# qucontrol/krotov

Hardware: AMD Instinct MI355X
Metric: state*timestep propagations/s (Krotov iterations/s in iterations_per_sec), 256-objective N=64 ensemble (higher is better)
Workload: dtype f64

## Files before the change

krotov_amd/csrc/kh_tile64q2.h:

```cpp
#pragma once

#include "kh_common.h"
#include "kh_generic.h"
#include "kh_tile64.h"

#define KH_Q2_THREADS 512
#ifdef KH_Q2_DPP_REDUCE
typedef KhLanes<false> KhQ2Lanes;
#else
typedef KhLanes<true> KhQ2Lanes;
#endif
#define KH_Q2_TILE_ELEMS (8 * KH_Q2_THREADS)

#ifdef KH_Q2_LDS_BROADCAST
constexpr bool KH_Q2_R16 = false;
#else
constexpr bool KH_Q2_R16 = true;
#endif

template <bool R16>
struct KhQ2Map;
template <>
struct KhQ2Map<false> {
    static __device__ __forceinline__ int half(int) { return 0; }
    static __device__ __forceinline__ int row_in(int wave, int lane) { return wave * 8 + KhQ2Lanes::row_in(lane); }
    static __device__ __forceinline__ int col(int, int lane, int j) { return KhQ2Lanes::cg(lane) + 8 * j; }
    static __device__ __forceinline__ int row_out(int wave, int lane) { return wave * 8 + KhQ2Lanes::row_out(lane); }
    static __device__ __forceinline__ bool writer(int lane) { return (lane & 7) == 0; }
    static __device__ __forceinline__ double rowsum(double v, double scale) { return KhQ2Lanes::rowsum(v, scale); }
};
template <>
struct KhQ2Map<true> {
    static __device__ __forceinline__ int half(int wave) { return KhLanesR16::half(wave); }
    static __device__ __forceinline__ int row_in(int wave, int lane) { return KhLanesR16::row_in(wave, lane); }
    static __device__ __forceinline__ int col(int wave, int lane, int j) { return KhLanesR16::col0(wave, lane) + j; }
    static __device__ __forceinline__ int row_out(int wave, int lane) { return KhLanesR16::row_out(wave, lane); }
    static __device__ __forceinline__ bool writer(int lane) { return KhLanesR16::writer(lane); }
    static __device__ __forceinline__ double rowsum(double v, double scale) { return KhLanesR16::rowsum(v, scale); }
};

struct KhQ2Lds {
    cplx *h0;
    cplx *p0;
    cplx (*buf)[2][KH_TILE_N];
    cplx *chib;
    cplx (*sbuf)[KH_TILE_N];
    double *red;
    double *D;
    double2 *inv2;
    double *deg;
};

__host__ __device__ inline size_t kh_q2_lds_bytes() {
    return (size_t)2 * KH_Q2_TILE_ELEMS * sizeof(cplx) + 7 * KH_TILE_N * sizeof(cplx) + (2 * 8 * 2 + 4) * sizeof(double) +
           (KH_MAX_DEGREE / 2 + 1) * sizeof(double2) + (KH_MAX_DEGREE + 2) * sizeof(double);
}

__device__ __forceinline__ KhQ2Lds kh_q2_carve(char *smem) {
    KhQ2Lds s;
    s.h0 = (cplx *)smem;
    s.p0 = s.h0 + KH_Q2_TILE_ELEMS;
    s.buf = (cplx(*)[2][KH_TILE_N])(s.p0 + KH_Q2_TILE_ELEMS);
    s.chib = (cplx *)(s.buf + 2);
    s.sbuf = (cplx(*)[KH_TILE_N])(s.chib + KH_TILE_N);
    s.red = (double *)(s.sbuf + 2);
    s.D = s.red + 2 * 8 * 2;
    s.inv2 = (double2 *)(s.D + 4);
    s.deg = (double *)(s.inv2 + KH_MAX_DEGREE / 2 + 1);
    return s;
}

template <bool R16>
__device__ __forceinline__ void kh_q2_load_tile(const cplx *op, int N, int wave, int lane, cplx (&t)[8]) {
    const int row = KhQ2Map<R16>::row_in(wave, lane);
#pragma unroll
    for (int j = 0; j < 8; ++j) {
        const int col = KhQ2Map<R16>::col(wave, lane, j);
        t[j] = (op != nullptr && row < N && col < N) ? op[(size_t)row * N + col] : c_make(0.0, 0.0);
    }
}

template <bool R16>
__device__ __forceinline__ void kh_q2_stage_tile(const cplx *op, int N, int wave, int lane, int tid, cplx *dst) {
    cplx t[8];
    kh_q2_load_tile<R16>(op, N, wave, lane, t);
#pragma unroll
    for (int j = 0; j < 8; ++j) dst[j * KH_Q2_THREADS + tid] = t[j];
}

__device__ __forceinline__ void kh_q2_load_rows(const KhSweepArgs &p, const KhQ2Lds &s, int m, int tid) {
    __syncthreads();
    if (tid < KH_Q2_ROWS) {
        const double *r = p.q2_rows + ((size_t)m * KH_Q2_ROWS + tid) * 2;
        s.inv2[tid] = make_double2(r[0], r[1]);
    }
    if (tid == KH_Q2_ROWS) s.inv2[KH_Q2_ROWS] = make_double2(p.q2_c0[m], 0.0);
    __syncthreads();
}

template <bool R16>
__device__ __forceinline__ cplx kh_q2_dot(const cplx (&t)[8], const cplx *x0, const cplx *x1, int wave, int lane) {
    cplx acc = c_make(0.0, 0.0);
    if constexpr (R16) {
        const int xi = KhLanesR16::x_index(wave, lane);
        const cplx xa = x0[xi], xb = x1[xi];
        KhLanesR16::dot8(acc, t, c_make(xa.x + xb.x, xa.y + xb.y));
    } else {
        const int cg = KhQ2Lanes::cg(lane);
        cplx xv[8];
#pragma unroll
        for (int j = 0; j < 8; ++j) xv[j] = x0[cg + 8 * j];
#pragma unroll
        for (int j = 0; j < 8; ++j) c_fma(acc, t[j], xv[j]);
    }
    return acc;
}
template <bool R16>
__device__ __forceinline__ cplx kh_q2_vec_at(const cplx (*v)[KH_TILE_N], int i) {
    cplx x = v[0][i];
    if constexpr (R16) {
        x.x += v[1][i].x;
        x.y += v[1][i].y;
    }
    return x;
}

__device__ __forceinline__ void kh_q2_build(const KhQ2Lds &s, int tid, double eps, const cplx (&h1)[8],
                                            const cplx (&p1)[8], const cplx (&p2)[8], cplx (&a)[8], cplx (&b)[8]) {
    const double eps2 = eps * eps;
#pragma unroll
    for (int j = 0; j < 8; ++j) {
        const cplx h0 = s.h0[j * KH_Q2_THREADS + tid];
        const cplx q0 = s.p0[j * KH_Q2_THREADS + tid];
        a[j].x = fma(eps, h1[j].x, h0.x);
        a[j].y = fma(eps, h1[j].y, h0.y);
        b[j].x = fma(eps2, p2[j].x, fma(eps, p1[j].x, q0.x));
        b[j].y = fma(eps2, p2[j].y, fma(eps, p1[j].y, q0.y));
    }
}

#define KH_Q2_REFRESH 64
__device__ __forceinline__ void kh_q2_restart_lds(const KhQ2Lds &s, int tid, cplx (&a)[8], cplx (&b)[8]) {
#pragma unroll
    for (int j = 0; j < 8; ++j) {
        a[j] = s.h0[j * KH_Q2_THREADS + tid];
        b[j] = s.p0[j * KH_Q2_THREADS + tid];
    }
}
__device__ __forceinline__ void kh_q2_advance_reg(double eps, double eps_prev, const cplx (&h1)[8], const cplx (&p1)[8],
                                                  const cplx (&p2)[8], cplx (&a)[8], cplx (&b)[8]) {
    const double e1 = eps - eps_prev, e2 = e1 * (eps + eps_prev);
#pragma unroll
    for (int j = 0; j < 8; ++j) {
        a[j].x = fma(e1, h1[j].x, a[j].x);
        a[j].y = fma(e1, h1[j].y, a[j].y);
        b[j].x = fma(e2, p2[j].x, fma(e1, p1[j].x, b[j].x));
        b[j].y = fma(e2, p2[j].y, fma(e1, p1[j].y, b[j].y));
    }
}

__device__ __forceinline__ void kh_q2_advance(const KhQ2Lds &s, int tid, double eps, double eps_prev, const cplx (&h1)[8],
                                              cplx (&a)[8], cplx (&b)[8]) {
    const double e1 = eps - eps_prev, e2 = e1 * (eps + eps_prev);
#pragma unroll
    for (int j = 0; j < 8; ++j) {
        const cplx q1 = s.h0[j * KH_Q2_THREADS + tid];
        const cplx q2 = s.p0[j * KH_Q2_THREADS + tid];
        a[j].x = fma(e1, h1[j].x, a[j].x);
        a[j].y = fma(e1, h1[j].y, a[j].y);
        b[j].x = fma(e2, q2.x, fma(e1, q1.x, b[j].x));
        b[j].y = fma(e2, q2.y, fma(e1, q1.y, b[j].y));
    }
}

template <bool R16, class Epilogue>
__device__ __forceinline__ int kh_q2_expm_action(const cplx (&a)[8], const cplx (&b)[8], cplx &state,
                                                 cplx (*buf)[2][KH_TILE_N], cplx (*sbuf)[KH_TILE_N], const double2 *inv2,
                                                 int &cur, cplx *store_in, int N, double fre, double fim,
                                                 double dt, int nsub, int m, bool odd, int wave, int lane,
                                                 Epilogue epilogue) {
    typedef KhQ2Map<R16> Map;
    const int row = Map::row_out(wave, lane), half = Map::half(wave);
    const bool writer = Map::writer(lane);
    const double h = nsub == 1 ? dt : dt / nsub;
    const double f2h2 = (fre * fre - fim * fim) * h * h;
    const int phases = (m + 1) >> 1;
    const bool no_last_b = odd && (m & 1);
    if (store_in != nullptr && wave == 0 && lane < N) {
        store_in[lane] = kh_q2_vec_at<R16>(buf[cur], lane);
    }
    for (int sub = 0; sub < nsub; ++sub) {
        const double hr = h * inv2[0].x, c0 = inv2[KH_Q2_ROWS].x;
        cplx sacc = c_make(hr * state.x, hr * state.y);
        state = c_make(c0 * state.x, c0 * state.y);
        if (phases == 1) {
            if (writer) sbuf[half][row] = sacc;
            __syncthreads();
        }
        for (int ph = 0; ph < phases; ++ph) {
            const bool last = (ph + 1 == phases);
            if (!(last && no_last_b)) {
                double c2, hn = 0.0;
                cplx yb;
                if constexpr (R16) {
                    const int xi = KhLanesR16::x_index(wave, lane);
                    const cplx x0 = buf[cur][0][xi], x1 = buf[cur][1][xi];
                    const double r2 = inv2[ph].y, r1n = inv2[ph + 1].x;
                    c2 = f2h2 * r2;
                    hn = h * r1n;
                    yb = c_make(0.0, 0.0);
                    KhLanesR16::dot8(yb, b, c_make(x0.x + x1.x, x0.y + x1.y));
                } else {
                    c2 = f2h2 * inv2[ph].y;
                    yb = kh_q2_dot<R16>(b, buf[cur][0], buf[cur][1], wave, lane);
                }
                const double t2x = Map::rowsum(yb.x, c2), t2y = Map::rowsum(yb.y, c2);
                state.x += t2x;
                state.y += t2y;
                if (!last) {
                    if constexpr (!R16) hn = h * inv2[ph + 1].x;
                    sacc.x = fma(hn, t2x, sacc.x);
                    sacc.y = fma(hn, t2y, sacc.y);
                    if (writer) {
                        buf[cur ^ 1][half][row] = c_make(t2x, t2y);
                        if (ph + 2 == phases) sbuf[half][row] = sacc;
                    }
                }
            }
            if (last) {
                __builtin_amdgcn_sched_barrier(0);
                const cplx ya = kh_q2_dot<R16>(a, sbuf[0], sbuf[1], wave, lane);
                const cplx odd_sum = c_mul(c_make(fre, fim), c_make(Map::rowsum(ya.x, 1.0), Map::rowsum(ya.y, 1.0)));
                state.x += odd_sum.x;
                state.y += odd_sum.y;
                if (writer) buf[cur ^ 1][half][row] = c_make(state.x, state.y);
                if (sub + 1 == nsub) epilogue();
            }
            __syncthreads();
            cur ^= 1;
        }
    }
    return nsub * (phases + (no_last_b ? 0 : 1));
}

template <bool R16>
__device__ __forceinline__ void kh_q2_sweep_store_body(const KhSweepArgs &p, const cplx *const *__restrict__ sq,
                                                       const double *__restrict__ pulses,
                                                       const cplx *__restrict__ state_in, cplx *__restrict__ store,
                                                       cplx *__restrict__ state_out, int direction, char *smem) {
    const KhQ2Lds s = kh_q2_carve(smem);
    const int tid = threadIdx.x, wave = tid >> 6, lane = tid & 63;
    if (tid <= KH_MAX_DEGREE) s.deg[tid] = p.q2_theta[tid];
    typedef KhQ2Map<R16> Map;
    const int row = Map::row_out(wave, lane);
    const int half = Map::half(wave);
    const bool writer = Map::writer(lane);
    const int N = p.N, nt = p.nt;
    double matvecs = 0.0;
    for (int k = blockIdx.x; k < p.K; k += gridDim.x) {
        const cplx *const *ops_k = p.ops + (size_t)k * 2;
        const cplx *const *sq_k = sq + (size_t)k * 3;
        __syncthreads();
        kh_q2_stage_tile<R16>(ops_k[0], N, wave, lane, tid, s.h0);
        kh_q2_stage_tile<R16>(sq_k[0], N, wave, lane, tid, s.p0);
        cplx h1[8], p1[8], p2[8];
        kh_q2_load_tile<R16>(ops_k[1], N, wave, lane, h1);
        kh_q2_load_tile<R16>(sq_k[1], N, wave, lane, p1);
        kh_q2_load_tile<R16>(sq_k[2], N, wave, lane, p2);
        const double nrm0 = p.op_norms[(size_t)k * 2], nrm1 = p.op_norms[(size_t)k * 2 + 1];

        cplx state = (row < N && half == 0) ? state_in[(size_t)k * N + row] : c_make(0.0, 0.0);
        int cur = 0;
        if (writer) s.buf[0][half][row] = state;
        __syncthreads();
        const int n0 = direction > 0 ? 0 : nt - 2;
        double eps_next = pulses[n0], dt_next = p.dt[n0];
        KhDegreeCache dc = {12, 1.0, 0.0};
        int m_rows = -1;
#ifdef KH_TIMING
        long long t_build = 0, t_phases = 0;
#endif
        cplx a[8], b[8];
        double eps_prev = 0.0;
        for (int step0 = 0; step0 < nt - 1; step0 += KH_Q2_REFRESH) {
        kh_q2_restart_lds(s, tid, a, b);
        eps_prev = 0.0;
        const int step_stop = step0 + KH_Q2_REFRESH < nt - 1 ? step0 + KH_Q2_REFRESH : nt - 1;
        for (int step = step0; step < step_stop; ++step) {
#ifdef KH_TIMING
            const long long tq0 = clock64();
#endif
            const int n = direction > 0 ? step : nt - 2 - step;
            const double eps = eps_next, dt = dt_next;
            if (step + 1 < nt - 1) {
                const int nn = direction > 0 ? n + 1 : n - 1;
                dt_next = p.dt[nn];
                eps_next = pulses[nn];
            }
            int nsub, m;
            kh_degree_cached((nrm0 + fabs(eps) * nrm1) * dt, s.deg, p.theta_max, p.inv_theta_max, dc, &nsub, &m);
            if (m != m_rows) {
                kh_q2_load_rows(p, s, m, tid);
                m_rows = m;
            }
            kh_q2_advance_reg(eps, eps_prev, h1, p1, p2, a, b);
            eps_prev = eps;
            cplx *store_in =
                store == nullptr ? nullptr : store + ((size_t)k * nt + (direction > 0 ? n : n + 1)) * N;
#ifdef KH_TIMING
            const long long tq1 = clock64();
            t_build += tq1 - tq0;
#endif
            matvecs += kh_q2_expm_action<R16>(a, b, state, s.buf, s.sbuf, s.inv2, cur, store_in, N, p.fre, p.fim, dt, nsub,
                                              m, p.q2_odd != 0, wave, lane, [] {});
#ifdef KH_TIMING
            t_phases += clock64() - tq1;
#endif
        }
        }
#ifdef KH_TIMING
        if (tid == 0 && k == 0 && p.stats != nullptr) {
            p.stats[1] = (double)t_build;
            p.stats[2] = (double)t_phases;
        }
#endif
        if (store != nullptr && wave == 0 && lane < N)
            store[((size_t)k * nt + (direction > 0 ? nt - 1 : 0)) * N + lane] = kh_q2_vec_at<R16>(s.buf[cur], lane);
        if (state_out != nullptr && wave == 0 && lane < N)
            state_out[(size_t)k * N + lane] = kh_q2_vec_at<R16>(s.buf[cur], lane);
    }
    if (tid == 0 && p.stats != nullptr) atomicAdd(p.stats, matvecs);
}

__global__ void __launch_bounds__(KH_Q2_THREADS)
kh_q2_sweep_store(KhSweepArgs p, const cplx *const *__restrict__ sq, const double *__restrict__ pulses,
                  const cplx *__restrict__ state_in, cplx *__restrict__ store, cplx *__restrict__ state_out,
                  int direction)
#if KH_DEFINES(KH_TU_Q2)
{
    extern __shared__ __attribute__((aligned(16))) char smem[];
    if (KH_Q2_R16 && !(direction > 0))
        kh_q2_sweep_store_body<true>(p, sq, pulses, state_in, store, state_out, direction, smem);
    else
        kh_q2_sweep_store_body<false>(p, sq, pulses, state_in, store, state_out, direction, smem);
}
#else
    ;
#endif

template <bool SO, bool ADJ, bool SINGLE = false>
__global__ void __launch_bounds__(KH_Q2_THREADS)
kh_q2_forward_update(KhSweepArgs p, const cplx *const *__restrict__ sq, KhUpdateArgs u, KhExchange ex) {
    static_assert(!(SO && ADJ), "the second-order bra depends on the new state");
#ifdef KH_Q2_NO_PREFETCH
    constexpr bool PREFETCH = false;
#else
    constexpr bool PREFETCH = !SO;
#endif
#ifdef KH_Q2_NARROW_POLL
    constexpr bool WIDE_POLL = false;
#else
    constexpr bool WIDE_POLL = true;
#endif
    if (u.n_dev != nullptr) {
        u.n_begin = *u.n_dev;
        u.n_end = u.n_begin + 1;
        if (u.n_begin >= p.nt - 1) return;
    }
    extern __shared__ __attribute__((aligned(16))) char smem[];
    const KhQ2Lds s = kh_q2_carve(smem);
    double(*red)[8][2] = (double(*)[8][2])s.red;
    double(*D_sh)[2] = (double(*)[2])s.D;
    const int tid = threadIdx.x, wave = tid >> 6, lane = tid & 63, cg = KhQ2Lanes::cg(lane);
    if (tid <= KH_MAX_DEGREE) s.deg[tid] = p.q2_theta[tid];
    const int row = wave * 8 + KhQ2Lanes::row_out(lane);
    if (wave < 4) __builtin_amdgcn_s_setprio(1);
    const bool writer = (lane & 7) == 0;
    const int N = p.N, nt = p.nt;
    const int k = blockIdx.x;
    double matvecs = 0.0;

    const cplx *const *ops_k = p.ops + (size_t)k * 2;
    const cplx *const *sq_k = sq + (size_t)k * 3;
    kh_q2_stage_tile<false>(sq_k[1], N, wave, lane, tid, s.h0);
    kh_q2_stage_tile<false>(sq_k[2], N, wave, lane, tid, s.p0);
    cplx h1[8], a[8], b[8];
    kh_q2_load_tile<false>(ops_k[1], N, wave, lane, h1);
    double eps_prev = 0.0;
    const double nrm0 = kh_uniform(p.op_norms[(size_t)k * 2]), nrm1 = kh_uniform(p.op_norms[(size_t)k * 2 + 1]);
    const double chi_norm = kh_uniform(u.chi_norms[k]);

    cplx state = row < N ? u.phi[(size_t)k * N + row] : c_make(0.0, 0.0);
    int cur = 0;
    if (writer) s.buf[0][0][row] = state;
    __syncthreads();

    double g_a_loc = 0.0;
    cplx chi = c_make(0.0, 0.0), prev = c_make(0.0, 0.0);
    double hs = 0.0;
    auto load_chi = [&](int n) {
        chi = row < N ? u.chi_store[((size_t)k * nt + n) * N + row] : c_make(0.0, 0.0);
        if constexpr (SO) {
            prev = row < N ? u.fw_prev[((size_t)k * nt + n) * N + row] : c_make(0.0, 0.0);
            hs = 0.5 * u.sigma[n] / chi_norm;
        }
    };

    auto partial_pieces = [&](int par) {
        cplx xv[8];
#pragma unroll
        for (int j = 0; j < 8; ++j) xv[j] = s.buf[cur][0][cg + 8 * j];
        cplx y = c_make(0.0, 0.0);
#pragma unroll
        for (int j = 0; j < 8; ++j) c_fma(y, h1[j], xv[j]);
        y.x = KhQ2Lanes::rowsum(y.x, 1.0);
        y.y = KhQ2Lanes::rowsum(y.y, 1.0);
        cplx ov = c_make(0.0, 0.0);
        cplx bra = chi;
        if constexpr (SO) bra = c_make(fma(hs, state.x - prev.x, chi.x), fma(hs, state.y - prev.y, chi.y));
        if (writer) c_fma_conj(ov, bra, y);
        const double v = KhQ2Lanes::writers_sum(u.mu_re * ov.y + u.mu_im * ov.x);
        if (lane == 0) red[par][wave][0] = v;
        matvecs += 1.0;
    };
    auto partial_total = [&](int par) {
        double acc = 0.0;
#pragma unroll
        for (int w = 0; w < 8; ++w) acc += red[par][w][0];
        return chi_norm * acc;
    };

    cplx w = c_make(0.0, 0.0);
    auto adjoint_side = [&]() {
        cplx xv[8];
#pragma unroll
        for (int j = 0; j < 8; ++j) xv[j] = s.chib[cg + 8 * j];
        cplx y = c_make(0.0, 0.0);
#pragma unroll
        for (int j = 0; j < 8; ++j) c_fma(y, h1[j], xv[j]);
        w.x = KhQ2Lanes::rowsum(y.x, u.adj_sign);
        w.y = KhQ2Lanes::rowsum(y.y, u.adj_sign);
        matvecs += 1.0;
    };

    if (u.n_begin < nt - 1) {
        load_chi(u.n_begin);
        partial_pieces(u.n_begin & 1);
    }
    if constexpr (ADJ) {
        if (u.n_begin + 1 < nt - 1) {
            load_chi(u.n_begin + 1);
            if (writer) s.chib[row] = chi;
        }
    }
    __syncthreads();

    double dt_next = kh_uniform(p.dt[u.n_begin]), guess_next = kh_uniform(u.guess[u.n_begin]),
           shape_next = kh_uniform(u.shape[u.n_begin]);
    const double lam = kh_uniform(u.lambda[0]);
    int m_rows = -1;
    double stepw_next = kh_uniform(shape_next / lam);
    KhDegreeCache dc = {12, 1.0, 0.0};

#ifdef KH_TIMING
    long long t_ex = 0, t_prop = 0, t_part = 0, t_coll = 0;
    const long long t_all0 = clock64();
#endif
    for (int nr = u.n_begin, n_stop; nr < u.n_end; nr = n_stop) {
    kh_q2_load_tile<false>(ops_k[0], N, wave, lane, a);
    kh_q2_load_tile<false>(sq_k[0], N, wave, lane, b);
    eps_prev = 0.0;
    n_stop = (nr / KH_Q2_REFRESH + 1) * KH_Q2_REFRESH;
    n_stop = n_stop < u.n_end ? n_stop : u.n_end;
    for (int n = nr; n < n_stop; ++n) {
        const int par = n & 1;
        if constexpr (!ADJ) {
            if (n + 1 < nt - 1) load_chi(n + 1);
        }
#ifdef KH_TIMING
        const long long tq0 = clock64();
#endif
        cplx q1[8], q2[8];
        {
            double part[1] = {0.0};
            if (wave == 0) {
                part[0] = partial_total(par);
#ifndef KH_Q2_X_NOEXCH
                kh_exchange_publish(ex, n, k, 1, lane, part);
#endif
            }
            if constexpr (PREFETCH) {
#pragma unroll
                for (int j = 0; j < 8; ++j) {
                    q1[j] = s.h0[j * KH_Q2_THREADS + tid];
                    q2[j] = s.p0[j * KH_Q2_THREADS + tid];
                }
            }
            if constexpr (ADJ) {
                if (n + 1 < nt - 1) adjoint_side();
            }
            if (wave == 0) {
                double D[1];
#ifdef KH_Q2_X_NOEXCH
                const bool ok = true;
                D[0] = part[0];
#else
#ifdef KH_TIMING
                const long long tc0 = clock64();
#endif
                const bool ok = kh_exchange_collect<1, KH_GATHER_CHUNKS, !SINGLE, WIDE_POLL>(ex, n, k, 1, lane, part, D);
#ifdef KH_TIMING
                t_coll += clock64() - tc0;
#endif
#endif
                if (lane == 0) {
                    D_sh[par][0] = D[0];
                    D_sh[par][1] = ok ? 1.0 : 0.0;
                }
            }
        }
        const double dt = dt_next, guess = guess_next, stepw = stepw_next;
        double dt_ld = 0.0, guess_ld = 0.0, shape_ld = 0.0;
        if (n + 1 < nt - 1) {
            dt_ld = p.dt[n + 1];
            guess_ld = u.guess[n + 1];
            shape_ld = u.shape[n + 1];
        }
        __syncthreads();
#ifdef KH_TIMING
        const long long tq1 = clock64();
        t_ex += tq1 - tq0;
#endif
        if (D_sh[par][1] == 0.0) return;
        const double d1 = D_sh[par][0];
        const double eps = kh_uniform(guess + stepw * d1);
        g_a_loc = kh_uniform(g_a_loc + stepw * (d1 * d1) * dt);
        dt_next = kh_uniform(dt_ld);
        guess_next = kh_uniform(guess_ld);
        shape_next = kh_uniform(shape_ld);
        if (k == 0 && tid == 0) u.opt[n] = eps;
        int nsub, m;
        kh_degree_cached((nrm0 + fabs(eps) * nrm1) * dt, s.deg, p.theta_max, p.inv_theta_max, dc, &nsub, &m);
        if (m != m_rows) {
            kh_q2_load_rows(p, s, m, tid);
            m_rows = m;
        }
        if constexpr (PREFETCH)
            kh_q2_advance_reg(eps, eps_prev, h1, q1, q2, a, b);
        else
            kh_q2_advance(s, tid, eps, eps_prev, h1, a, b);
        eps_prev = eps;
        stepw_next = kh_uniform(shape_next / lam);
        cplx *fw_out = nullptr;
        if constexpr (SO) fw_out = u.fw_store + ((size_t)k * nt + n) * N;
        if constexpr (ADJ) {
            if (n + 2 < nt - 1) load_chi(n + 2);
            auto epilogue = [&] {
                if (n + 1 < nt - 1) {
                    cplx ov = c_make(0.0, 0.0);
                    if (writer) c_fma_conj(ov, w, state);
                    const double v = KhQ2Lanes::writers_sum(u.mu_re * ov.y + u.mu_im * ov.x);
                    if (lane == 0) red[(n + 1) & 1][wave][0] = v;
                    if (n + 2 < nt - 1 && writer) s.chib[row] = chi;
                }
            };
#ifdef KH_Q2_X_NOPHASES
            epilogue();
            __syncthreads();
#else
            matvecs += kh_q2_expm_action<false>(a, b, state, s.buf, s.sbuf, s.inv2, cur, fw_out, N, p.fre, p.fim, dt, nsub, m,
                                         p.q2_odd != 0, wave, lane, epilogue);
#endif
        } else {
            matvecs += kh_q2_expm_action<false>(a, b, state, s.buf, s.sbuf, s.inv2, cur, fw_out, N, p.fre, p.fim, dt, nsub, m,
                                         p.q2_odd != 0, wave, lane, [] {});
        }
#ifdef KH_TIMING
        const long long tq2 = clock64();
        t_prop += tq2 - tq1;
#endif
        if constexpr (!ADJ) {
            if (n + 1 < nt - 1) {
                partial_pieces((n + 1) & 1);
                __syncthreads();
            }
        }
#ifdef KH_TIMING
        t_part += clock64() - tq2;
#endif
    }
    }
#ifdef KH_TIMING
    if (tid == 0 && k == 0 && p.stats != nullptr) {
        p.stats[1] = (double)t_ex;
        p.stats[2] = (double)t_prop;
        p.stats[3] = (double)t_coll;
    }
#endif
    if (wave == 0 && lane < N) {
        u.phi[(size_t)k * N + lane] = s.buf[cur][0][lane];
        if constexpr (SO) u.fw_store[((size_t)k * nt + u.n_end) * N + lane] = s.buf[cur][0][lane];
    }
    if (k == 0 && tid == 0) u.g_a[0] = g_a_loc;
    if (tid == 0 && p.stats != nullptr) atomicAdd(p.stats, matvecs);
}

__global__ void kh_q2_product(const cplx *__restrict__ X, const cplx *__restrict__ Y, cplx *__restrict__ C, int N,
                              int symmetrize)
#if KH_DEFINES(KH_TU_MAIN)
{
    for (int idx = blockIdx.x * blockDim.x + threadIdx.x; idx < N * N; idx += gridDim.x * blockDim.x) {
        const int i = idx / N, j = idx % N;
        cplx acc = c_make(0.0, 0.0);
        for (int q = 0; q < N; ++q) c_fma(acc, X[(size_t)i * N + q], Y[(size_t)q * N + j]);
        if (symmetrize)
            for (int q = 0; q < N; ++q) c_fma(acc, Y[(size_t)i * N + q], X[(size_t)q * N + j]);
        C[idx] = acc;
    }
}
#else
    ;
#endif
```

Before: 71.10 million.

## Add compile-time-unrolled static expm phase path with precomputed LDS coefficients

Adds a template-recursive KhQ2Static path that fully unrolls the polynomial-expm phases for single-substep cases with degree 9 to 14. Per-phase scalar coefficients are formed once per dt change into a small LDS coef table, so the runtime phase loop and its per-phase coefficient arithmetic go away. The path is on by default for the backward sweep (R16 layout) and off for the update kernel. It also adds uniformity hints and opaque-index asm to shape codegen, at the cost of code size and extra template instantiations.

Result: no change. 71.69 million (median of 6 runs) (+0.8%).

```diff
diff --git a/krotov_amd/csrc/kh_tile64q2.h b/krotov_amd/csrc/kh_tile64q2.h
--- a/krotov_amd/csrc/kh_tile64q2.h
+++ b/krotov_amd/csrc/kh_tile64q2.h
@@ -11,6 +11,7 @@
 typedef KhLanes<true> KhQ2Lanes;
 #endif
 #define KH_Q2_TILE_ELEMS (8 * KH_Q2_THREADS)
+#define KH_Q2_SPEC_PMAX 7
 
 #ifdef KH_Q2_LDS_BROADCAST
 constexpr bool KH_Q2_R16 = false;
@@ -49,11 +50,13 @@
     double *D;
     double2 *inv2;
     double *deg;
+    double2 *coef;
 };
 
 __host__ __device__ inline size_t kh_q2_lds_bytes() {
     return (size_t)2 * KH_Q2_TILE_ELEMS * sizeof(cplx) + 7 * KH_TILE_N * sizeof(cplx) + (2 * 8 * 2 + 4) * sizeof(double) +
-           (KH_MAX_DEGREE / 2 + 1) * sizeof(double2) + (KH_MAX_DEGREE + 2) * sizeof(double);
+           (KH_MAX_DEGREE / 2 + 1) * sizeof(double2) + (KH_MAX_DEGREE + 2) * sizeof(double) +
+           (KH_Q2_SPEC_PMAX + 1) * sizeof(double2);
 }
 
 __device__ __forceinline__ KhQ2Lds kh_q2_carve(char *smem) {
@@ -67,6 +70,9 @@
     s.D = s.red + 2 * 8 * 2;
     s.inv2 = (double2 *)(s.D + 4);
     s.deg = (double *)(s.inv2 + KH_MAX_DEGREE / 2 + 1);
+    int zero = 0;
+    asm("" : "+v"(zero));
+    s.coef = (double2 *)(s.deg + KH_MAX_DEGREE + 2) + zero;
     return s;
 }
 
@@ -243,6 +249,155 @@
     return nsub * (phases + (no_last_b ? 0 : 1));
 }
 
+__device__ __forceinline__ void kh_q2_form_coef(const KhQ2Lds &s, double fre, double fim, double dt, int tid) {
+    const double h = dt;
+    const double f2h2 = (fre * fre - fim * fim) * h * h;
+    if (tid < KH_Q2_SPEC_PMAX) s.coef[tid] = make_double2(f2h2 * s.inv2[tid].y, h * s.inv2[tid + 1].x);
+    if (tid == KH_Q2_SPEC_PMAX) s.coef[tid] = make_double2(s.inv2[KH_Q2_ROWS].x, h * s.inv2[0].x);
+    __syncthreads();
+}
+
+#ifndef KH_Q2_STATIC_BACKWARD
+#define KH_Q2_STATIC_BACKWARD 1
+#endif
+#ifndef KH_Q2_STATIC_UPDATE
+#define KH_Q2_STATIC_UPDATE 0
+#endif
+
+template <bool R16, int P, bool NO_LAST_B, int CUR>
+struct KhQ2Static {
+    typedef KhQ2Map<R16> Map;
+    struct Ctx {
+        const cplx (*rd)[2][KH_TILE_N];
+        cplx (*wr)[2][KH_TILE_N];
+        cplx *swr;
+        bool writer;
+    };
+
+    template <int PH, class Epilogue>
+    static __device__ __forceinline__ void phase(const cplx (&a)[8], const cplx (&b)[8], cplx &state, cplx &sacc,
+                                                 const Ctx &cx, const cplx (*sbuf)[KH_TILE_N], const double2 *coef,
+                                                 cplx *store_in, int N, double fre, double fim, int wave, int lane,
+                                                 double c2_in, Epilogue &epilogue) {
+        constexpr bool last = PH + 1 == P;
+        constexpr int in = CUR ^ (PH & 1), out = in ^ 1;
+        double c2_next = 0.0;
+        double2 c0hr = make_double2(0.0, 0.0);
+        if constexpr (!(last && NO_LAST_B)) {
+            cplx yb = c_make(0.0, 0.0);
+            double c2 = c2_in, hn = 0.0;
+            if constexpr (R16) {
+                const cplx x0 = cx.rd[in][0][0], x1 = cx.rd[in][1][0];
+                __builtin_amdgcn_sched_barrier(0);
+                const double2 cf = coef[PH];
+                if constexpr (PH == 0) c0hr = coef[KH_Q2_SPEC_PMAX];
+                c2 = cf.x;
+                hn = cf.y;
+                const cplx x = c_make(x0.x + x1.x, x0.y + x1.y);
+                KhLanesR16::dot8(yb, b, x);
+                if constexpr (PH == 0) {
+                    if (store_in != nullptr && wave < 2) {
+                        const int xi = KhLanesR16::x_index(wave, lane);
+                        if ((lane & 8) == 0 && xi < N) store_in[xi] = x;
+                    }
+                }
+            } else {
+                cplx xv[8];
+#pragma unroll
+                for (int j = 0; j < 8; ++j) xv[j] = cx.rd[in][0][8 * j];
+#pragma unroll
+                for (int j = 0; j < 8; ++j) c_fma(yb, b[j], xv[j]);
+                if constexpr (!last) {
+                    hn = coef[PH].y;
+                    if constexpr (!(PH + 2 == P && NO_LAST_B)) c2_next = coef[PH + 1].x;
+                    if constexpr (PH == 0) c0hr = coef[KH_Q2_SPEC_PMAX];
+                }
+            }
+            const double t2x = Map::rowsum(yb.x, c2), t2y = Map::rowsum(yb.y, c2);
+            if constexpr (!last) {
+                if (cx.writer) cx.wr[out][0][0] = c_make(t2x, t2y);
+                if constexpr (PH == 0) {
+                    sacc = c_make(c0hr.y * state.x, c0hr.y * state.y);
+                    state = c_make(c0hr.x * state.x, c0hr.x * state.y);
+                    asm volatile("" : "+v"(state.x), "+v"(state.y));
+                }
+                sacc.x = fma(hn, t2x, sacc.x);
+                sacc.y = fma(hn, t2y, sacc.y);
+                asm volatile("" : "+v"(sacc.x), "+v"(sacc.y));
+                if constexpr (PH + 2 == P) {
+                    if (cx.writer) *cx.swr = sacc;
+                }
+            }
+            state.x += t2x;
+            state.y += t2y;
+        }
+        if constexpr (last) {
+            __builtin_amdgcn_sched_barrier(0);
+            const cplx ya = kh_q2_dot<R16>(a, sbuf[0], sbuf[1], wave, lane);
+            const cplx odd_sum = c_mul(c_make(fre, fim), c_make(Map::rowsum(ya.x, 1.0), Map::rowsum(ya.y, 1.0)));
+            state.x += odd_sum.x;
+            state.y += odd_sum.y;
+            if (cx.writer) cx.wr[out][0][0] = c_make(state.x, state.y);
+            epilogue();
+        }
+        __syncthreads();
+        if constexpr (!last)
+            phase<PH + 1>(a, b, state, sacc, cx, sbuf, coef, store_in, N, fre, fim, wave, lane, c2_next, epilogue);
+    }
+
+    template <class Epilogue>
+    static __device__ __forceinline__ void run(const cplx (&a)[8], const cplx (&b)[8], cplx &state,
+                                               cplx (*buf)[2][KH_TILE_N], cplx (*sbuf)[KH_TILE_N], const double2 *coef,
+                                               cplx *store_in, int N, double fre, double fim, int wave, int lane,
+                                               Epilogue &epilogue) {
+        const int row = Map::row_out(wave, lane), half = Map::half(wave);
+        const int xi = R16 ? KhLanesR16::x_index(wave, lane) : KhQ2Lanes::cg(lane);
+        Ctx cx;
+        cx.rd = (const cplx(*)[2][KH_TILE_N])(&buf[0][0][xi]);
+        cx.wr = (cplx(*)[2][KH_TILE_N])(&buf[0][half][row]);
+        cx.swr = &sbuf[half][row];
+        cx.writer = Map::writer(lane);
+        if constexpr (!R16) {
+            if (store_in != nullptr && wave == 0 && lane < N) store_in[lane] = buf[CUR][0][lane];
+        }
+        cplx sacc;
+        phase<0>(a, b, state, sacc, cx, sbuf, coef, store_in, N, fre, fim, wave, lane, R16 ? 0.0 : coef[0].x, epilogue);
+    }
+};
+
+template <bool R16, bool STATIC, class Epilogue>
+__device__ __forceinline__ int kh_q2_expm_step(const cplx (&a)[8], const cplx (&b)[8], cplx &state,
+                                               cplx (*buf)[2][KH_TILE_N], cplx (*sbuf)[KH_TILE_N], const double2 *inv2,
+                                               const double2 *coef, int &cur, cplx *store_in, int N, double fre, double fim,
+                                               double dt, int nsub, int m, bool odd, int wave, int lane,
+                                               Epilogue epilogue) {
+#define KH_Q2_STATIC_CASE(PHASES, NLB)                                                                                  \
+    if (cur == 0)                                                                                                       \
+        KhQ2Static<R16, PHASES, NLB, 0>::run(a, b, state, buf, sbuf, coef, store_in, N, fre, fim, wave, lane, epilogue); \
+    else                                                                                                                \
+        KhQ2Static<R16, PHASES, NLB, 1>::run(a, b, state, buf, sbuf, coef, store_in, N, fre, fim, wave, lane, epilogue); \
+    cur ^= (PHASES & 1);                                                                                                \
+    return PHASES + (NLB ? 0 : 1);
+    if (STATIC && nsub == 1) {
+        switch (odd ? m : ((m + 1) & ~1)) {
+        case 9: KH_Q2_STATIC_CASE(5, true)
+        case 10: KH_Q2_STATIC_CASE(5, false)
+        case 11: KH_Q2_STATIC_CASE(6, true)
+        case 12: KH_Q2_STATIC_CASE(6, false)
+        case 13: KH_Q2_STATIC_CASE(7, true)
+        case 14: KH_Q2_STATIC_CASE(7, false)
+        default: break;
+        }
+    }
+#undef KH_Q2_STATIC_CASE
+    return kh_q2_expm_action<R16>(a, b, state, buf, sbuf, inv2, cur, store_in, N, fre, fim, dt, nsub, m, odd, wave, lane,
+                                  epilogue);
+}
+
+__device__ __forceinline__ int kh_q2_opaque(int i) {
+    asm volatile("" : "+v"(i));
+    return i;
+}
 template <bool R16>
 __device__ __forceinline__ void kh_q2_sweep_store_body(const KhSweepArgs &p, const cplx *const *__restrict__ sq,
                                                        const double *__restrict__ pulses,
@@ -255,8 +410,9 @@
     const int row = Map::row_out(wave, lane);
     const int half = Map::half(wave);
     const bool writer = Map::writer(lane);
+    constexpr bool STATIC_STEP = R16 && KH_Q2_STATIC_BACKWARD != 0;
     const int N = p.N, nt = p.nt;
-    double matvecs = 0.0;
+    long long matvecs = 0;
     for (int k = blockIdx.x; k < p.K; k += gridDim.x) {
         const cplx *const *ops_k = p.ops + (size_t)k * 2;
         const cplx *const *sq_k = sq + (size_t)k * 3;
@@ -267,9 +423,9 @@
         kh_q2_load_tile<R16>(ops_k[1], N, wave, lane, h1);
         kh_q2_load_tile<R16>(sq_k[1], N, wave, lane, p1);
         kh_q2_load_tile<R16>(sq_k[2], N, wave, lane, p2);
-        const double nrm0 = p.op_norms[(size_t)k * 2], nrm1 = p.op_norms[(size_t)k * 2 + 1];
-
-        cplx state = (row < N && half == 0) ? state_in[(size_t)k * N + row] : c_make(0.0, 0.0);
+        const double nrm0 = kh_uniform(p.op_norms[(size_t)k * 2]), nrm1 = kh_uniform(p.op_norms[(size_t)k * 2 + 1]);
+
+        cplx state = (row < N && half == 0) ? state_in[(size_t)k * N + kh_q2_opaque(row)] : c_make(0.0, 0.0);
         int cur = 0;
         if (writer) s.buf[0][half][row] = state;
         __syncthreads();
@@ -277,6 +433,7 @@
         double eps_next = pulses[n0], dt_next = p.dt[n0];
         KhDegreeCache dc = {12, 1.0, 0.0};
         int m_rows = -1;
+        double dt_rows = 0.0;
 #ifdef KH_TIMING
         long long t_build = 0, t_phases = 0;
 #endif
@@ -291,7 +448,7 @@
             const long long tq0 = clock64();
 #endif
             const int n = direction > 0 ? step : nt - 2 - step;
-            const double eps = eps_next, dt = dt_next;
+            const double eps = kh_uniform(eps_next), dt = kh_uniform(dt_next);
             if (step + 1 < nt - 1) {
                 const int nn = direction > 0 ? n + 1 : n - 1;
                 dt_next = p.dt[nn];
@@ -299,8 +456,14 @@
             }
             int nsub, m;
             kh_degree_cached((nrm0 + fabs(eps) * nrm1) * dt, s.deg, p.theta_max, p.inv_theta_max, dc, &nsub, &m);
-            if (m != m_rows) {
-                kh_q2_load_rows(p, s, m, tid);
+            dc.lo = kh_uniform(dc.lo);
+            dc.hi = kh_uniform(dc.hi);
+            if (m != m_rows || (STATIC_STEP && dt != dt_rows)) {
+                if (m != m_rows) kh_q2_load_rows(p, s, m, tid);
+                if constexpr (STATIC_STEP) {
+                    kh_q2_form_coef(s, p.fre, p.fim, dt, tid);
+                    dt_rows = kh_uniform(dt);
+                }
                 m_rows = m;
             }
             kh_q2_advance_reg(eps, eps_prev, h1, p1, p2, a, b);
@@ -311,8 +474,12 @@
             const long long tq1 = clock64();
             t_build += tq1 - tq0;
 #endif
-            matvecs += kh_q2_expm_action<R16>(a, b, state, s.buf, s.sbuf, s.inv2, cur, store_in, N, p.fre, p.fim, dt, nsub,
-                                              m, p.q2_odd != 0, wave, lane, [] {});
+            if constexpr (STATIC_STEP)
+                matvecs += kh_q2_expm_step<R16, true>(a, b, state, s.buf, s.sbuf, s.inv2, s.coef, cur, store_in, N, p.fre,
+                                                      p.fim, dt, nsub, m, p.q2_odd != 0, wave, lane, [] {});
+            else
+                matvecs += kh_q2_expm_action<R16>(a, b, state, s.buf, s.sbuf, s.inv2, cur, store_in, N, p.fre, p.fim, dt, nsub,
+                                                  m, p.q2_odd != 0, wave, lane, [] {});
 #ifdef KH_TIMING
             t_phases += clock64() - tq1;
 #endif
@@ -325,11 +492,11 @@
         }
 #endif
         if (store != nullptr && wave == 0 && lane < N)
-            store[((size_t)k * nt + (direction > 0 ? nt - 1 : 0)) * N + lane] = kh_q2_vec_at<R16>(s.buf[cur], lane);
+            store[((size_t)k * nt + (direction > 0 ? nt - 1 : 0)) * N + kh_q2_opaque(lane)] = kh_q2_vec_at<R16>(s.buf[cur], lane);
         if (state_out != nullptr && wave == 0 && lane < N)
-            state_out[(size_t)k * N + lane] = kh_q2_vec_at<R16>(s.buf[cur], lane);
-    }
-    if (tid == 0 && p.stats != nullptr) atomicAdd(p.stats, matvecs);
+            state_out[(size_t)k * N + kh_q2_opaque(lane)] = kh_q2_vec_at<R16>(s.buf[cur], lane);
+    }
+    if (tid == 0 && p.stats != nullptr) atomicAdd(p.stats, (double)matvecs);
 }
 
 __global__ void __launch_bounds__(KH_Q2_THREADS)
@@ -459,6 +626,8 @@
            shape_next = kh_uniform(u.shape[u.n_begin]);
     const double lam = kh_uniform(u.lambda[0]);
     int m_rows = -1;
+    constexpr bool STATIC_STEP = KH_Q2_STATIC_UPDATE != 0;
+    double dt_rows = 0.0;
     double stepw_next = kh_uniform(shape_next / lam);
     KhDegreeCache dc = {12, 1.0, 0.0};
 
@@ -541,8 +710,16 @@
         if (k == 0 && tid == 0) u.opt[n] = eps;
         int nsub, m;
         kh_degree_cached((nrm0 + fabs(eps) * nrm1) * dt, s.deg, p.theta_max, p.inv_theta_max, dc, &nsub, &m);
-        if (m != m_rows) {
-            kh_q2_load_rows(p, s, m, tid);
+        if constexpr (STATIC_STEP) {
+            dc.lo = kh_uniform(dc.lo);
+            dc.hi = kh_uniform(dc.hi);
+        }
+        if (m != m_rows || (STATIC_STEP && dt != dt_rows)) {
+            if (m != m_rows) kh_q2_load_rows(p, s, m, tid);
+            if constexpr (STATIC_STEP) {
+                kh_q2_form_coef(s, p.fre, p.fim, dt, tid);
+                dt_rows = kh_uniform(dt);
+            }
             m_rows = m;
         }
         if constexpr (PREFETCH)
@@ -568,11 +745,11 @@
             epilogue();
             __syncthreads();
 #else
-            matvecs += kh_q2_expm_action<false>(a, b, state, s.buf, s.sbuf, s.inv2, cur, fw_out, N, p.fre, p.fim, dt, nsub, m,
+            matvecs += kh_q2_expm_step<false, STATIC_STEP>(a, b, state, s.buf, s.sbuf, s.inv2, s.coef, cur, fw_out, N, p.fre, p.fim, dt, nsub, m,
                                          p.q2_odd != 0, wave, lane, epilogue);
 #endif
         } else {
-            matvecs += kh_q2_expm_action<false>(a, b, state, s.buf, s.sbuf, s.inv2, cur, fw_out, N, p.fre, p.fim, dt, nsub, m,
+            matvecs += kh_q2_expm_step<false, STATIC_STEP>(a, b, state, s.buf, s.sbuf, s.inv2, s.coef, cur, fw_out, N, p.fre, p.fim, dt, nsub, m,
                                          p.q2_odd != 0, wave, lane, [] {});
         }
 #ifdef KH_TIMING
```
